# ForJadeForest/DistillCLIP

Hardware: AMD Instinct MI355X
Metric: image-text pairs/sec (distill step) (higher is better)
Workload: dtype bf16; 1 GPU; l_clip.yaml dual distill: ViT-B/32 CLIP teacher -> weight-shared ViT(6x768,24h,R2) + text(4x768,12h,R2) students, 224px/77tok, losses out_l1+out_cos+0.1*cos_diff, fwd+loss+bwd+AdamW; global_batch=512, batch_per_gpu=512, parallelism=dp1, gradient_exchange=none, negatives=local (reference training_step semantics), optimizer_in_step=True, teacher_residual=fp16, saved_gelu_derivative=u8 fixed point, clock_probe=True

## Files before the change

### distillclip_amd/csrc/layernorm.hip

```cpp
#include <stdlib.h>
#include "common.h"

namespace {

constexpr int LN_MAXV = 4;

template <int NV, int OUT, bool X_F16>
__global__ __launch_bounds__(256) void ln_fwd_kernel(const void* __restrict__ x, int64_t ldx, const int* __restrict__ ridx,
                                                     const float* __restrict__ gamma, const float* __restrict__ beta,
                                                     void* __restrict__ y, int64_t ldy, float* __restrict__ mean,
                                                     float* __restrict__ rstd, int M, int D, float eps) {
    const int lane = threadIdx.x & 63;
    const int row = blockIdx.x * 4 + (threadIdx.x >> 6);
    if (row >= M) return;
    const int64_t src = ridx ? ridx[row] : row;
    float4 v[NV];
    float s = 0.f;
#pragma unroll
    for (int i = 0; i < NV; ++i) {
        const int c = (i * 64 + lane) * 4;
        v[i] = float4{0.f, 0.f, 0.f, 0.f};
        if (c < D) {
            if (X_F16) {
                const f16x4 h = *(const f16x4*)((const _Float16*)x + src * ldx + c);
                v[i] = float4{(float)h[0], (float)h[1], (float)h[2], (float)h[3]};
            } else {
                v[i] = *(const float4*)((const float*)x + src * ldx + c);
            }
        }
        s += (v[i].x + v[i].y) + (v[i].z + v[i].w);
    }
    const float mu = wave_sum(s) / D;
    float q = 0.f;
#pragma unroll
    for (int i = 0; i < NV; ++i) {
        const int c = (i * 64 + lane) * 4;
        if (c < D) {
            const float a = v[i].x - mu, b = v[i].y - mu, cc = v[i].z - mu, d = v[i].w - mu;
            q += (a * a + b * b) + (cc * cc + d * d);
        }
    }
    const float rs = rsqrtf(wave_sum(q) / D + eps);
    if (lane == 0) {
        if (mean) mean[row] = mu;
        if (rstd) rstd[row] = rs;
    }
#pragma unroll
    for (int i = 0; i < NV; ++i) {
        const int c = (i * 64 + lane) * 4;
        if (c < D) {
            const float4 g = *(const float4*)(gamma + c), b = *(const float4*)(beta + c);
            const float o0 = (v[i].x - mu) * rs * g.x + b.x, o1 = (v[i].y - mu) * rs * g.y + b.y;
            const float o2 = (v[i].z - mu) * rs * g.z + b.z, o3 = (v[i].w - mu) * rs * g.w + b.w;
            if (OUT == 1) {
                *(float4*)((float*)y + (int64_t)row * ldy + c) = float4{o0, o1, o2, o3};
            } else if (OUT == 2) {
                *(f16x4*)((_Float16*)y + (int64_t)row * ldy + c) = f16x4{(_Float16)o0, (_Float16)o1, (_Float16)o2, (_Float16)o3};
            } else {
                bf16x4 o = {f2bf(o0), f2bf(o1), f2bf(o2), f2bf(o3)};
                *(bf16x4*)((bf16_t*)y + (int64_t)row * ldy + c) = o;
            }
        }
    }
}

template <int NV, bool DY_F32>
__global__ __launch_bounds__(512) void ln_bwd_kernel(const void* __restrict__ dy, int64_t lddy, const float* __restrict__ x,
                                                     int64_t ldx, const int* __restrict__ ridx,
                                                     const float* __restrict__ gamma, const float* __restrict__ mean,
                                                     const float* __restrict__ rstd, float* __restrict__ dx_acc,
                                                     int64_t lddx, bf16_t* __restrict__ dx_bf16, int64_t lddb,
                                                     float* __restrict__ dgamma, float* __restrict__ dbeta, float* __restrict__ colsum, int M, int D) {
    constexpr int NW = 8, DP = NV * 256;
    extern __shared__ float red_[];
    float (*red)[NW][DP] = (float (*)[NW][DP])red_;
    const int lane = threadIdx.x & 63, wave = threadIdx.x >> 6;
    float4 dg[NV], db[NV], gm[NV], cs[NV];
#pragma unroll
    for (int i = 0; i < NV; ++i) {
        dg[i] = db[i] = cs[i] = float4{0.f, 0.f, 0.f, 0.f};
        const int c = (i * 64 + lane) * 4;
        gm[i] = c < D ? *(const float4*)(gamma + c) : float4{0.f, 0.f, 0.f, 0.f};
    }
    struct Raw {
        float4 x[NV], a[NV], d[NV];
        float mu, rs;
        int64_t src;
        int row;
    };
    auto issue = [&](int row, Raw& r) {
        r.row = row;
        r.src = ridx ? ridx[row] : row;
        r.mu = mean[row];
        r.rs = rstd[row];
#pragma unroll
        for (int i = 0; i < NV; ++i) {
            const int c = (i * 64 + lane) * 4;
            r.x[i] = r.a[i] = r.d[i] = float4{0.f, 0.f, 0.f, 0.f};
            if (c < D) {
                r.x[i] = *(const float4*)(x + r.src * ldx + c);
                r.a[i] = *(const float4*)(dx_acc + r.src * lddx + c);
                if (DY_F32) r.d[i] = *(const float4*)((const float*)dy + (int64_t)row * lddy + c);
                else {
                    const bf16x4 t = *(const bf16x4*)((const bf16_t*)dy + (int64_t)row * lddy + c);
                    union { bf16x4 h; float2 f; } u; u.h = t;
                    r.d[i].x = u.f.x; r.d[i].y = u.f.y;
                }
            }
        }
    };
    auto process = [&](const Raw& r) {
        float4 xh[NV], g[NV];
        float s1 = 0.f, s2 = 0.f;
#pragma unroll
        for (int i = 0; i < NV; ++i) {
            const int c = (i * 64 + lane) * 4;
            xh[i] = g[i] = float4{0.f, 0.f, 0.f, 0.f};
            if (c < D) {
                float4 d;
                if (DY_F32) d = r.d[i];
                else {
                    union { bf16x4 h; float2 f; } u; u.f = float2{r.d[i].x, r.d[i].y};
                    d = float4{bf2f(u.h[0]), bf2f(u.h[1]), bf2f(u.h[2]), bf2f(u.h[3])};
                }
                const float4 xv = r.x[i];
                xh[i] = float4{(xv.x - r.mu) * r.rs, (xv.y - r.mu) * r.rs, (xv.z - r.mu) * r.rs, (xv.w - r.mu) * r.rs};
                g[i] = float4{d.x * gm[i].x, d.y * gm[i].y, d.z * gm[i].z, d.w * gm[i].w};
                s1 += (g[i].x + g[i].y) + (g[i].z + g[i].w);
                s2 += (g[i].x * xh[i].x + g[i].y * xh[i].y) + (g[i].z * xh[i].z + g[i].w * xh[i].w);
                dg[i].x += d.x * xh[i].x; dg[i].y += d.y * xh[i].y; dg[i].z += d.z * xh[i].z; dg[i].w += d.w * xh[i].w;
                db[i].x += d.x; db[i].y += d.y; db[i].z += d.z; db[i].w += d.w;
            }
        }
        const float c1 = wave_sum(s1) / D, c2 = wave_sum(s2) / D;
#pragma unroll
        for (int i = 0; i < NV; ++i) {
            const int c = (i * 64 + lane) * 4;
            if (c < D) {
                float* o = dx_acc + r.src * lddx + c;
                float4 a = r.a[i];
                a.x += r.rs * (g[i].x - c1 - xh[i].x * c2);
                a.y += r.rs * (g[i].y - c1 - xh[i].y * c2);
                a.z += r.rs * (g[i].z - c1 - xh[i].z * c2);
                a.w += r.rs * (g[i].w - c1 - xh[i].w * c2);
                *(float4*)o = a;
                cs[i].x += a.x; cs[i].y += a.y; cs[i].z += a.z; cs[i].w += a.w;
                if (dx_bf16) {
                    bf16x4 bq = {f2bf(a.x), f2bf(a.y), f2bf(a.z), f2bf(a.w)};
                    *(bf16x4*)(dx_bf16 + r.src * lddb + c) = bq;
                }
            }
        }
    };
    const int stride = gridDim.x * NW;
    Raw ra, rb;
    int row = blockIdx.x * NW + wave;
    if (row < M) issue(row, ra);
    while (row < M) {
        int nrow = row + stride;
        if (nrow < M) issue(nrow, rb);
        process(ra);
        row = nrow;
        if (row >= M) break;
        nrow = row + stride;
        if (nrow < M) issue(nrow, ra);
        process(rb);
        row = nrow;
    }
#pragma unroll
    for (int i = 0; i < NV; ++i) {
        const int c = (i * 64 + lane) * 4;
        *(float4*)&red[0][wave][c] = dg[i];
        *(float4*)&red[1][wave][c] = db[i];
        *(float4*)&red[2][wave][c] = cs[i];
    }
    __syncthreads();
    for (int c = threadIdx.x; c < D; c += 64 * NW) {
        float a = 0.f, b = 0.f, k = 0.f;
#pragma unroll
        for (int w = 0; w < NW; ++w) { a += red[0][w][c]; b += red[1][w][c]; k += red[2][w][c]; }
        if (dgamma) unsafeAtomicAdd(dgamma + c, a);
        if (dbeta) unsafeAtomicAdd(dbeta + c, b);
        if (colsum) unsafeAtomicAdd(colsum + c, k);
    }
}

}

#define LN_DISPATCH(NVV, ...)                     \
    switch (NVV) {                                \
        case 1: { constexpr int NV = 1; __VA_ARGS__; break; } \
        case 2: { constexpr int NV = 2; __VA_ARGS__; break; } \
        case 3: { constexpr int NV = 3; __VA_ARGS__; break; } \
        default: { constexpr int NV = 4; __VA_ARGS__; break; } \
    }

static int ln_fwd_launch(const void* x, int x_f16, int64_t ldx, const int32_t* row_index, const float* gamma, const float* beta, void* y,
                         int64_t ldy, int out, float* mean, float* rstd, int64_t M, int64_t D, float eps, void* stream, const char* who) {
    DCLIP_REQUIRE(x && gamma && beta && y, "%s: null operand", who);
    DCLIP_REQUIRE(M > 0 && D > 0 && D % 4 == 0 && D <= 1024, "%s: need 0 < D <= 1024, D %% 4 == 0 (D=%ld)", who, (long)D);
    DCLIP_REQUIRE(ldx % 4 == 0 && ldy % 4 == 0 && ((uintptr_t)x % (x_f16 ? 8 : 16)) == 0, "%s: row strides must be multiples of 4, rows 8- (fp16) / 16-byte aligned", who);
    DCLIP_REQUIRE(out >= 0 && out <= 2 && (out != 2 || x_f16), "%s: output dtype 0 bf16 / 1 f32 (/ 2 f16 with f16 input)", who);
    const int nv = (int)((D + 255) / 256);
    const dim3 grid((unsigned)((M + 3) / 4));
    hipStream_t st = (hipStream_t)stream;
    TraceScope tr(DCLIP_TRACE_LAYERNORM, 8.0 * (double)M * D, (double)M * D * ((x_f16 ? 2.0 : 4.0) + (out == 1 ? 4.0 : 2.0)), stream);
#define LN_GO(OUTV, XH) hipLaunchKernelGGL((ln_fwd_kernel<NV, OUTV, XH>), grid, dim3(256), 0, st, x, ldx, row_index, gamma, beta, y, ldy, mean, rstd, (int)M, (int)D, eps)
    LN_DISPATCH(nv,
        if (x_f16) { if (out == 2) LN_GO(2, true); else if (out == 1) LN_GO(1, true); else LN_GO(0, true); }
        else { if (out == 1) LN_GO(1, false); else LN_GO(0, false); });
#undef LN_GO
    return dclip_check_launch(who);
}

extern "C" int dclip_layernorm_fwd(const float* x, int64_t ldx, const int32_t* row_index, const float* gamma,
                                   const float* beta, void* y, int64_t ldy, int out_f32, float* mean, float* rstd,
                                   int64_t M, int64_t D, float eps, void* stream) {
    return ln_fwd_launch(x, 0, ldx, row_index, gamma, beta, y, ldy, out_f32 ? 1 : 0, mean, rstd, M, D, eps, stream, "dclip_layernorm_fwd");
}

extern "C" int dclip_layernorm_fwd_f16(const void* x, int64_t ldx, const int32_t* row_index, const float* gamma,
                                       const float* beta, void* y, int64_t ldy, int out_dtype, float* mean, float* rstd,
                                       int64_t M, int64_t D, float eps, void* stream) {
    return ln_fwd_launch(x, 1, ldx, row_index, gamma, beta, y, ldy, out_dtype, mean, rstd, M, D, eps, stream, "dclip_layernorm_fwd_f16");
}

extern "C" int dclip_layernorm_bwd(const void* dy, int64_t lddy, int dy_f32, const float* x, int64_t ldx,
                                   const int32_t* row_index, const float* gamma, const float* mean, const float* rstd,
                                   float* dx_acc, int64_t lddx, void* dx_bf16, int64_t lddb, float* dgamma, float* dbeta,
                                   float* colsum_acc, int64_t M, int64_t D, void* stream) {
    DCLIP_REQUIRE(dy && x && gamma && mean && rstd && dx_acc, "dclip_layernorm_bwd: null operand");
    DCLIP_REQUIRE(M > 0 && D > 0 && D % 4 == 0 && D <= 1024, "dclip_layernorm_bwd: need 0 < D <= 1024, D %% 4 == 0 (D=%ld)", (long)D);
    const int nv = (int)((D + 255) / 256);
    int blocks = (int)((M + 7) / 8);
    if (blocks > 256) blocks = 256;
    TraceScope tr(DCLIP_TRACE_LN_BWD, 12.0 * (double)M * D, (double)M * D * ((dy_f32 ? 4.0 : 2.0) + 12.0 + (dx_bf16 ? 2.0 : 0.0)), stream, (int)M, (int)D, 0, 0);
    hipStream_t st = (hipStream_t)stream;
    LN_DISPATCH(nv,
        if (dy_f32) hipLaunchKernelGGL((ln_bwd_kernel<NV, true>), dim3(blocks), dim3(512), (size_t)3 * 8 * NV * 256 * 4, st, dy, lddy, x, ldx, row_index, gamma, mean, rstd, dx_acc, lddx, (bf16_t*)dx_bf16, lddb, dgamma, dbeta, colsum_acc, (int)M, (int)D);
        else hipLaunchKernelGGL((ln_bwd_kernel<NV, false>), dim3(blocks), dim3(512), (size_t)3 * 8 * NV * 256 * 4, st, dy, lddy, x, ldx, row_index, gamma, mean, rstd, dx_acc, lddx, (bf16_t*)dx_bf16, lddb, dgamma, dbeta, colsum_acc, (int)M, (int)D));
    return dclip_check_launch("dclip_layernorm_bwd");
}
```

Measured before the change: 18300 pairs/s.

## Make LayerNorm forward persistent with software-pipelined row prefetch

Turns the LayerNorm forward kernel into a grid-stride persistent kernel capped at a few blocks per CU. Each wave issues the next row's global loads with inline asm and explicit vmcnt waits before it processes the current row, and gamma/beta are loaded once per wave instead of once per row. A FULL template variant drops the column bounds checks when D is a multiple of 256. This aims to hide load latency and cut per-row launch and parameter reload cost, but it adds register pressure and relies on hand-counted vmcnt values that are fragile.

```diff
diff --git a/distillclip_amd/csrc/layernorm.hip b/distillclip_amd/csrc/layernorm.hip
--- a/distillclip_amd/csrc/layernorm.hip
+++ b/distillclip_amd/csrc/layernorm.hip
@@ -1,67 +1,141 @@
 #include <stdlib.h>
+#include <atomic>
+#include <type_traits>
 #include "common.h"
 
 namespace {
 
 constexpr int LN_MAXV = 4;
 
-template <int NV, int OUT, bool X_F16>
+template <class T> __device__ __forceinline__ void vm_load(T& dst, const void* p) {
+    if constexpr (sizeof(T) == 16) asm volatile("global_load_dwordx4 %0, %1, off" : "=v"(dst) : "v"(p));
+    else asm volatile("global_load_dwordx2 %0, %1, off" : "=v"(dst) : "v"(p));
+}
+template <int N, class T, int K> __device__ __forceinline__ void vm_wait(T (&a)[K]) {
+    static_assert(K >= 1 && K <= 4 && N >= 0 && N < 64, "vmcnt is a 6-bit count");
+    if constexpr (K == 1) asm volatile("s_waitcnt vmcnt(%[n])" : "+v"(a[0]) : [n] "i"(N));
+    else if constexpr (K == 2) asm volatile("s_waitcnt vmcnt(%[n])" : "+v"(a[0]), "+v"(a[1]) : [n] "i"(N));
+    else if constexpr (K == 3) asm volatile("s_waitcnt vmcnt(%[n])" : "+v"(a[0]), "+v"(a[1]), "+v"(a[2]) : [n] "i"(N));
+    else asm volatile("s_waitcnt vmcnt(%[n])" : "+v"(a[0]), "+v"(a[1]), "+v"(a[2]), "+v"(a[3]) : [n] "i"(N));
+}
+
+template <int I, int N, class F> __device__ __forceinline__ void static_for(F&& f) {
+    if constexpr (I < N) { f(std::integral_constant<int, I>{}); static_for<I + 1, N>(f); }
+}
+
+constexpr int LN_AHEAD = 1;
+constexpr int LN_FWD_WAVES = 4;
+constexpr int LN_FWD_BLOCKS_PER_CU = 4;
+
+template <int NV, int OUT, bool X_F16, bool FULL>
 __global__ __launch_bounds__(256) void ln_fwd_kernel(const void* __restrict__ x, int64_t ldx, const int* __restrict__ ridx,
                                                      const float* __restrict__ gamma, const float* __restrict__ beta,
                                                      void* __restrict__ y, int64_t ldy, float* __restrict__ mean,
                                                      float* __restrict__ rstd, int M, int D, float eps) {
+    constexpr int AHEAD = LN_AHEAD, NB = AHEAD + 1;
     const int lane = threadIdx.x & 63;
-    const int row = blockIdx.x * 4 + (threadIdx.x >> 6);
+    const int wave = __builtin_amdgcn_readfirstlane(threadIdx.x >> 6);
+    const int64_t stride = (int64_t)gridDim.x * LN_FWD_WAVES;
+    int64_t row = (int64_t)blockIdx.x * LN_FWD_WAVES + wave;
     if (row >= M) return;
-    const int64_t src = ridx ? ridx[row] : row;
-    float4 v[NV];
-    float s = 0.f;
-#pragma unroll
-    for (int i = 0; i < NV; ++i) {
-        const int c = (i * 64 + lane) * 4;
-        v[i] = float4{0.f, 0.f, 0.f, 0.f};
-        if (c < D) {
-            if (X_F16) {
-                const f16x4 h = *(const f16x4*)((const _Float16*)x + src * ldx + c);
-                v[i] = float4{(float)h[0], (float)h[1], (float)h[2], (float)h[3]};
-            } else {
-                v[i] = *(const float4*)((const float*)x + src * ldx + c);
-            }
-        }
-        s += (v[i].x + v[i].y) + (v[i].z + v[i].w);
-    }
-    const float mu = wave_sum(s) / D;
-    float q = 0.f;
-#pragma unroll
-    for (int i = 0; i < NV; ++i) {
-        const int c = (i * 64 + lane) * 4;
-        if (c < D) {
-            const float a = v[i].x - mu, b = v[i].y - mu, cc = v[i].z - mu, d = v[i].w - mu;
-            q += (a * a + b * b) + (cc * cc + d * d);
-        }
-    }
-    const float rs = rsqrtf(wave_sum(q) / D + eps);
-    if (lane == 0) {
-        if (mean) mean[row] = mu;
-        if (rstd) rstd[row] = rs;
-    }
-#pragma unroll
-    for (int i = 0; i < NV; ++i) {
-        const int c = (i * 64 + lane) * 4;
-        if (c < D) {
-            const float4 g = *(const float4*)(gamma + c), b = *(const float4*)(beta + c);
-            const float o0 = (v[i].x - mu) * rs * g.x + b.x, o1 = (v[i].y - mu) * rs * g.y + b.y;
-            const float o2 = (v[i].z - mu) * rs * g.z + b.z, o3 = (v[i].w - mu) * rs * g.w + b.w;
-            if (OUT == 1) {
-                *(float4*)((float*)y + (int64_t)row * ldy + c) = float4{o0, o1, o2, o3};
-            } else if (OUT == 2) {
-                *(f16x4*)((_Float16*)y + (int64_t)row * ldy + c) = f16x4{(_Float16)o0, (_Float16)o1, (_Float16)o2, (_Float16)o3};
-            } else {
-                bf16x4 o = {f2bf(o0), f2bf(o1), f2bf(o2), f2bf(o3)};
-                *(bf16x4*)((bf16_t*)y + (int64_t)row * ldy + c) = o;
-            }
-        }
-    }
+    using XV = typename std::conditional<X_F16, f16x4, f32x4>::type;
+    struct Raw { XV x[NV]; };
+    using XT = typename std::conditional<X_F16, _Float16, float>::type;
+    int col[NV];
+#pragma unroll
+    for (int i = 0; i < NV; ++i) col[i] = FULL ? (i * 64 + lane) * 4 : min((i * 64 + lane) * 4, D - 4);
+    auto issue = [&](int64_t r, Raw& raw) {
+        const int64_t src = ridx ? ridx[r] : r;
+#pragma unroll
+        for (int i = 0; i < NV; ++i) vm_load(raw.x[i], (const XT*)x + src * ldx + col[i]);
+    };
+    f32x4 gm[NV], bt[NV];
+    Raw buf[NB];
+    auto open = [&]() {
+#pragma unroll
+        for (int i = 0; i < NV; ++i) { vm_load(gm[i], gamma + col[i]); vm_load(bt[i], beta + col[i]); }
+        issue(row, buf[0]);
+        vm_wait<NV>(gm);
+        vm_wait<NV>(bt);
+    };
+    auto process = [&](Raw& raw, int64_t r, auto ahead) {
+        vm_wait<decltype(ahead)::value * NV>(raw.x);
+        float4 v[NV];
+        float s = 0.f;
+#pragma unroll
+        for (int i = 0; i < NV; ++i) {
+            const int c = (i * 64 + lane) * 4;
+            v[i] = float4{0.f, 0.f, 0.f, 0.f};
+            if (FULL || c < D) {
+                if constexpr (X_F16) v[i] = float4{(float)raw.x[i][0], (float)raw.x[i][1], (float)raw.x[i][2], (float)raw.x[i][3]};
+                else v[i] = float4{raw.x[i][0], raw.x[i][1], raw.x[i][2], raw.x[i][3]};
+            }
+            s += (v[i].x + v[i].y) + (v[i].z + v[i].w);
+        }
+        const float mu = wave_sum(s) / D;
+        float q = 0.f;
+#pragma unroll
+        for (int i = 0; i < NV; ++i) {
+            const int c = (i * 64 + lane) * 4;
+            if (FULL || c < D) {
+                const float a = v[i].x - mu, b = v[i].y - mu, cc = v[i].z - mu, d = v[i].w - mu;
+                q += (a * a + b * b) + (cc * cc + d * d);
+            }
+        }
+        const float rs = rsqrtf(wave_sum(q) / D + eps);
+        if (lane == 0) {
+            if (mean) mean[r] = mu;
+            if (rstd) rstd[r] = rs;
+        }
+#pragma unroll
+        for (int i = 0; i < NV; ++i) {
+            const int c = (i * 64 + lane) * 4;
+            if (FULL || c < D) {
+                const f32x4 g = gm[i], b = bt[i];
+                const float o0 = (v[i].x - mu) * rs * g.x + b.x, o1 = (v[i].y - mu) * rs * g.y + b.y;
+                const float o2 = (v[i].z - mu) * rs * g.z + b.z, o3 = (v[i].w - mu) * rs * g.w + b.w;
+                if (OUT == 1) {
+                    *(float4*)((float*)y + r * ldy + c) = float4{o0, o1, o2, o3};
+                } else if (OUT == 2) {
+                    *(f16x4*)((_Float16*)y + r * ldy + c) = f16x4{(_Float16)o0, (_Float16)o1, (_Float16)o2, (_Float16)o3};
+                } else {
+                    bf16x4 o = {f2bf(o0), f2bf(o1), f2bf(o2), f2bf(o3)};
+                    *(bf16x4*)((bf16_t*)y + r * ldy + c) = o;
+                }
+            }
+        }
+    };
+    if (row + AHEAD * stride >= M) {
+        open();
+#pragma unroll
+        for (int p = 1; p < AHEAD; ++p)
+            if (row + p * stride < M) issue(row + p * stride, buf[p]);
+#pragma unroll
+        for (int p = 0; p < AHEAD; ++p)
+            if (row + p * stride < M) process(buf[p], row + p * stride, std::integral_constant<int, 0>{});
+        return;
+    }
+    open();
+#pragma unroll
+    for (int p = 1; p < AHEAD; ++p) issue(row + p * stride, buf[p]);
+    int phase = 0;
+    for (bool more = true; more;) {
+#pragma unroll
+        for (int k = 0; k < NB; ++k) {
+            const int64_t nrow = row + AHEAD * stride;
+            if (nrow >= M) { phase = k; more = false; break; }
+            issue(nrow, buf[(k + AHEAD) % NB]);
+            process(buf[k], row, std::integral_constant<int, AHEAD>{});
+            row += stride;
+        }
+    }
+    static_for<0, AHEAD>([&](auto j) {
+        constexpr int J = decltype(j)::value;
+#pragma unroll
+        for (int k = 0; k < NB; ++k)
+            if ((phase + J) % NB == k) process(buf[k], row, std::integral_constant<int, AHEAD - 1 - J>{});
+        row += stride;
+    });
 }
 
 template <int NV, bool DY_F32>
@@ -195,6 +269,23 @@
         default: { constexpr int NV = 4; __VA_ARGS__; break; } \
     }
 
+static int ln_cu_count() {
+    static std::atomic<int> cus[64];
+    int dev = 0;
+    if (hipGetDevice(&dev) != hipSuccess || dev < 0 || dev >= 64) dev = 0;
+    int n = cus[dev].load(std::memory_order_relaxed);
+    if (n == 0) {
+        if (hipDeviceGetAttribute(&n, hipDeviceAttributeMultiprocessorCount, dev) != hipSuccess || n <= 0) n = 256;
+        cus[dev].store(n, std::memory_order_relaxed);
+    }
+    return n;
+}
+
+static int ln_fwd_block_cap() {
+    static const int v = [] { const char* e = getenv("DCLIP_LN_BLOCKS"); return e ? atoi(e) : 0; }();
+    return v;
+}
+
 static int ln_fwd_launch(const void* x, int x_f16, int64_t ldx, const int32_t* row_index, const float* gamma, const float* beta, void* y,
                          int64_t ldy, int out, float* mean, float* rstd, int64_t M, int64_t D, float eps, void* stream, const char* who) {
     DCLIP_REQUIRE(x && gamma && beta && y, "%s: null operand", who);
@@ -202,10 +293,17 @@
     DCLIP_REQUIRE(ldx % 4 == 0 && ldy % 4 == 0 && ((uintptr_t)x % (x_f16 ? 8 : 16)) == 0, "%s: row strides must be multiples of 4, rows 8- (fp16) / 16-byte aligned", who);
     DCLIP_REQUIRE(out >= 0 && out <= 2 && (out != 2 || x_f16), "%s: output dtype 0 bf16 / 1 f32 (/ 2 f16 with f16 input)", who);
     const int nv = (int)((D + 255) / 256);
-    const dim3 grid((unsigned)((M + 3) / 4));
+    int64_t blocks = (M + LN_FWD_WAVES - 1) / LN_FWD_WAVES;
+    const int64_t cap = ln_fwd_block_cap() > 0 ? ln_fwd_block_cap() : (int64_t)ln_cu_count() * LN_FWD_BLOCKS_PER_CU;
+    if (blocks > cap) blocks = cap;
+    const dim3 grid((unsigned)blocks);
     hipStream_t st = (hipStream_t)stream;
     TraceScope tr(DCLIP_TRACE_LAYERNORM, 8.0 * (double)M * D, (double)M * D * ((x_f16 ? 2.0 : 4.0) + (out == 1 ? 4.0 : 2.0)), stream);
-#define LN_GO(OUTV, XH) hipLaunchKernelGGL((ln_fwd_kernel<NV, OUTV, XH>), grid, dim3(256), 0, st, x, ldx, row_index, gamma, beta, y, ldy, mean, rstd, (int)M, (int)D, eps)
+#define LN_GO(OUTV, XH)                                                                                                                                   \
+    do {                                                                                                                                                  \
+        if (D == NV * 256) hipLaunchKernelGGL((ln_fwd_kernel<NV, OUTV, XH, true>), grid, dim3(256), 0, st, x, ldx, row_index, gamma, beta, y, ldy, mean, rstd, (int)M, (int)D, eps); \
+        else hipLaunchKernelGGL((ln_fwd_kernel<NV, OUTV, XH, false>), grid, dim3(256), 0, st, x, ldx, row_index, gamma, beta, y, ldy, mean, rstd, (int)M, (int)D, eps);            \
+    } while (0)
     LN_DISPATCH(nv,
         if (x_f16) { if (out == 2) LN_GO(2, true); else if (out == 1) LN_GO(1, true); else LN_GO(0, true); }
         else { if (out == 1) LN_GO(1, false); else LN_GO(0, false); });
```

After: 18450 pairs/s, median of 6. No clear change (+0.8%).
